# sekelle/SPH-EXA

Measured on AMD Instinct MI355X. Metric: particle-updates/sec (whole node), Sedov -n 400 and Evrard+gravity -n 200, higher is better.
Workload: dtype fp64 coordinates + fp32 hydro (reference precision mix); 1 GPU; model=sedov -n 400 --prop ve (64000000 particles), global_batch=64000000, seq_len=1, parallelism=sfc-domain-decomposition x1, ranks=1, backend=none, leaf_capacity=512

## Files before the change

### sphexa_amd/csrc/hip/bind_hip.cpp

```cpp
#include <array>
#include <stdexcept>
#include <vector>

#include <pybind11/pybind11.h>
#include <pybind11/stl.h>

#include "hip_api.h"

namespace py = pybind11;
using namespace sphx;
using namespace sphx::hip;

namespace
{
using BoxArr   = std::array<double, 9>;
using ConstArr = std::array<double, 16>;
using Ptr      = uintptr_t;

template<class T>
T* P(Ptr p)
{
    return reinterpret_cast<T*>(p);
}

// ... 322 lines not shown
    m.def("chunk_cap", []() { return kChunkCap; });
    m.def("packed_table_region", [](int64_t groups, unsigned ngmax) { return packedTableRegion(groups, ngmax); });

    m.def("xmass",
          [](int64_t first, int64_t last, const ConstArr& c, const BoxArr& box, Ptr nidx, Ptr nc, Ptr x, Ptr y, Ptr z,
             Ptr h, Ptr mm, Ptr wh, Ptr xm, int64_t ntot, Ptr rec, Ptr s, int inDone, Ptr out)
          {
              auto sc = toConsts(c);
              xmass(nbr(first, last, nidx, nc, sc), sc, toBox(box), ntot, P<double>(x), P<double>(y), P<double>(z),
                    P<float>(h), P<float>(mm), P<float>(wh), P<void>(rec), P<float>(xm), St(s), inDone, P<void>(out));
          },
          py::arg("first"), py::arg("last"), py::arg("c"), py::arg("box"), py::arg("nidx"), py::arg("nc"),
          py::arg("x"), py::arg("y"), py::arg("z"), py::arg("h"), py::arg("mm"), py::arg("wh"), py::arg("xm"),
          py::arg("ntot"), py::arg("rec"), py::arg("s"), py::arg("inDone") = 0, py::arg("out") = 0);
    m.def("ve_def_gradh",
          [](int64_t first, int64_t last, const ConstArr& c, const BoxArr& box, Ptr nidx, Ptr nc, Ptr x, Ptr y, Ptr z,
             Ptr h, Ptr mm, Ptr wh, Ptr whd, Ptr xm, Ptr kx, Ptr gradh, int64_t ntot, Ptr rec, Ptr s, double mUniform,
             int inDone, Ptr out, Ptr vx, Ptr vy, Ptr vz, Ptr eosTemp, Ptr eosPrho, Ptr eosC, Ptr eosRho, Ptr eosP)
          {
              auto sc = toConsts(c);
              veDefGradh(nbr(first, last, nidx, nc, sc), sc, toBox(box), ntot, P<double>(x), P<double>(y),
                         P<double>(z), P<float>(h), P<float>(mm), P<float>(wh), P<float>(whd), P<float>(xm),
                         P<void>(rec), P<float>(kx), P<float>(gradh), float(mUniform), St(s), inDone, P<void>(out),
                         P<float>(vx), P<float>(vy), P<float>(vz), P<double>(eosTemp), P<float>(eosPrho),
                         P<float>(eosC), P<float>(eosRho), P<float>(eosP));
          },
          py::arg("first"), py::arg("last"), py::arg("c"), py::arg("box"), py::arg("nidx"), py::arg("nc"),
          py::arg("x"), py::arg("y"), py::arg("z"), py::arg("h"), py::arg("mm"), py::arg("wh"), py::arg("whd"),
          py::arg("xm"), py::arg("kx"), py::arg("gradh"), py::arg("ntot"), py::arg("rec"), py::arg("s"),
          py::arg("mUniform"), py::arg("inDone") = 0, py::arg("out") = 0, py::arg("vx") = 0, py::arg("vy") = 0,
          py::arg("vz") = 0, py::arg("eosTemp") = 0, py::arg("eosPrho") = 0, py::arg("eosC") = 0,
          py::arg("eosRho") = 0, py::arg("eosP") = 0);
    m.def("set_staged", [](unsigned mask) { setStaged(mask); },
          "pair loops that run LDS-staged: bit 0 XMass, 1 Gradh, 2 IAD, 3 AV, 4 momentum (hydro.hip, staged.h)");
    m.def("staged_mask", []() { return stagedMask(); });
    m.def("set_list_masks", [](bool on) { setListMasks(on); },
          "store the per-slot staged-source masks in the list tables even without a staged loop (tests)");
    m.def("set_pair_paths", [](bool kernelFixed, bool momBuf) { setPairPaths(kernelFixed, momBuf); },
          "pair-loop instances: the compile-time sinc^6 kernel function and the momentum loop's 32-bit buffer gathers "
          "(defaults on; tests compare them with the generic instances)", py::arg("kernel_fixed"), py::arg("mom_buf"));
    m.def("set_pair_block", [](int block) { setPairBlock(block); },
          "threads per block of the fixed-point pair loops: 512 (8 target groups sharing a CU's L1) or 256");
    m.def("eos_ve", [](int64_t first, int64_t last, const ConstArr& c, Ptr temp, Ptr mm, Ptr kx, Ptr xm, Ptr gradh,
                       Ptr prho, Ptr cc, Ptr rho, Ptr p, Ptr s)
          {
              eosVe(first, last, toConsts(c), P<double>(temp), P<float>(mm), P<float>(kx), P<float>(xm),
                    P<float>(gradh), P<float>(prho), P<float>(cc), P<float>(rho), P<float>(p), St(s));
          });
    m.def("eos_polytropic", [](int64_t first, int64_t last, Ptr kx, Ptr xm, Ptr mm, Ptr p, Ptr c, Ptr s)
          { eosPolytropic(first, last, P<float>(kx), P<float>(xm), P<float>(mm), P<float>(p), P<float>(c), St(s)); });
    m.def("eos_std", [](int64_t first, int64_t last, const ConstArr& c, Ptr temp, Ptr mm, Ptr rho, Ptr p, Ptr cc,
                        Ptr s)
          {
              eosStd(first, last, toConsts(c), P<double>(temp), P<float>(mm), P<float>(rho), P<float>(p),
                     P<float>(cc), St(s));
          });
    m.def("iad", [](int64_t first, int64_t last, const ConstArr& c, const BoxArr& box, Ptr nidx, Ptr nc, Ptr x, Ptr y,
                    Ptr z, Ptr h, Ptr wh, Ptr numer, Ptr denom, const std::array<Ptr, 6>& cij, int64_t ntot, Ptr rec,
                    Ptr s)
          {
              auto sc = toConsts(c);
              auto cp = six(cij);
              iad(nbr(first, last, nidx, nc, sc), sc, toBox(box), ntot, P<double>(x), P<double>(y), P<double>(z),
                  P<float>(h), P<float>(wh), P<float>(numer), P<float>(denom), P<void>(rec), cp.data(), St(s));
          });
    m.def("iad_divv_curlv",
          [](int64_t first, int64_t last, const ConstArr& c, const BoxArr& box, Ptr nidx, Ptr nc, Ptr x, Ptr y, Ptr z,
             Ptr vx, Ptr vy, Ptr vz, Ptr h, const std::array<Ptr, 6>& cij, Ptr wh, Ptr kx, Ptr xm, Ptr divv,
             Ptr curlv, const std::array<Ptr, 6>& dV, int64_t ntot, Ptr rec, Ptr s, Ptr avS, int inDone, Ptr avOut,
             Ptr momOut, Ptr cs, Ptr mm, Ptr prho, int momSplit)
// ... 270 lines not shown
```

### sphexa_amd/csrc/hip/hip_api.h

```cpp
#pragma once

#include <cstdint>
#include <vector>

#include <hip/hip_runtime.h>

#include "sphx/box.hpp"
#include "sphx/cooling.hpp"
#include "sphx/sph_math.hpp"

namespace sphx::hip
{

struct NsTree
{
    const int32_t* child;
    const int32_t* n2l;
    const int32_t* ns;
    const int32_t* ne;
    const double* center;
    const double* half;
};

struct NbrArgs
// ... 107 lines not shown
void leafBoxesFused(const int32_t* n2l, int64_t N, const int32_t* ns, const int32_t* ne, const double* x,
                    const double* y, const double* z, const int32_t* child, const int32_t* parents, double* center,
                    double* half, unsigned* cnt, hipStream_t s);
void leafBoxes(const int32_t* n2l, int64_t N, const int32_t* ns, const int32_t* ne, const double* x,
               const double* y, const double* z, const float* h, double factor, double* center, double* half,
               hipStream_t s);
void upsweepBoxes(int64_t a, int64_t b, const int32_t* n2l, const int32_t* child, double* center, double* half,
                  hipStream_t s);
void markInBoxes(int64_t nb, const double* bc, const double* bh, const int32_t* child, const int32_t* n2l,
                 const int32_t* ns, const int32_t* ne, const double* center, const double* half, const double* x,
                 const double* y, const double* z, const Box& box, uint8_t* flags, hipStream_t s);

size_t neighborScratchBytes(int64_t n, unsigned ngmax);
struct SplitPredict
{
    const uint64_t* keys = nullptr;
    const unsigned long long* predIn = nullptr;
    unsigned long long* predOut = nullptr;
    int32_t* flags = nullptr;
    int stamp = 0;
    int cap = 0;
    unsigned long long* listCount = nullptr;
    int32_t* list = nullptr;
    int mark = 1;
};
void findNeighbors(int64_t first, int64_t last, const double* x, const double* y, const double* z, float* h,
                   const NsTree& t, const Box& box, unsigned ng0, unsigned ngmax, int32_t* nidx, int home,
                   int ovStride, int32_t* nc, int iterateH, unsigned long long* stats, void* scratch,
                   int testFrontCap, const float* m, int64_t ntot, void* rec, hipStream_t s, const SplitPredict& sp = SplitPredict{});
void setPairBlock(int block);
void setPairPaths(bool kernelFixed, bool momBuf);
void setStaged(unsigned mask);
unsigned stagedMask();
void setListMasks(bool on);
bool listMasksForced();
void packPosQ(int64_t n, const double* x, const double* y, const double* z, const float* m, const QFrame& q,
              SrcPosQ* out, hipStream_t s);
int neighborRowStripes();
void rowPlan(int64_t groups, unsigned ngmax, const int32_t* tab, int home, unsigned long long* over, hipStream_t s);

struct MomFields
{
    const double *x, *y, *z;
    const float *vx, *vy, *vz, *h, *m, *prho, *c;
    const float* cij[6];
    const float *kx, *xm, *alpha;
    const float* dV[6];
};

struct StdFields
{
    const double *x, *y, *z;
    const float *vx, *vy, *vz, *h, *m, *rho, *p, *c;
    const float* cij[6];
};

void xmass(const NbrArgs& a, const SphConsts& sc, const Box& box, int64_t ntot, const double* x, const double* y,
           const double* z, const float* h, const float* m, const float* wh, void* rec, float* xm, hipStream_t s,
           int inDone = 0, void* xmOut = nullptr);
void veDefGradh(const NbrArgs& a, const SphConsts& sc, const Box& box, int64_t ntot, const double* x,
                const double* y, const double* z, const float* h, const float* m, const float* wh, const float* whd,
                const float* xm, void* rec, float* kx, float* gradh, float mUniform, hipStream_t s, int inDone = 0,
                void* iadOut = nullptr, const float* vx = nullptr, const float* vy = nullptr,
                const float* vz = nullptr, const double* eosTemp = nullptr, float* eosPrho = nullptr,
                float* eosC = nullptr, float* eosRho = nullptr, float* eosP = nullptr);
void eosPolytropic(int64_t first, int64_t last, const float* kx, const float* xm, const float* m, float* p, float* c,
                   hipStream_t s);
// ... 106 lines not shown
```

### sphexa_amd/csrc/hip/hydro.hip

```cpp
#include <cfloat>
#include <cstdlib>
#include <type_traits>

#include "common.h"
#include "hip_api.h"
#include "sphx/sph_math.hpp"
#include "staged.h"

namespace sphx::hip
{

#ifndef SPHX_PAIR_BLOCK
#define SPHX_PAIR_BLOCK 256
#endif
constexpr int kBlock = SPHX_PAIR_BLOCK;

template<int B = kBlock>
__device__ __forceinline__ bool targetOf(const NbrArgs& a, int64_t& i, PackedLane& pl, unsigned& n)
{
    __shared__ uint32_t ctabAll[B / 64][kChunkCap];
    unsigned lb     = xcdRemap(blockIdx.x, gridDim.x);
    int64_t t       = int64_t(lb) * B + threadIdx.x;
    i               = a.first + t;
    const int64_t g = t >> 6;
// ... 78 lines not shown
{
    return CoopLoader<R>{rec, waveTile<R>(blockTile), unsigned(self)};
}

inline NbrArgs withTot(NbrArgs a, int64_t ntot)
{
    a.ntot = unsigned(ntot);
    return a;
}

inline unsigned gridT(const NbrArgs& a, int block = kBlock) { return gridFor(a.last - a.first, block); }

static int g_pairBlock = kBlock;
#ifndef SPHX_AV_BLOCK
#define SPHX_AV_BLOCK 640
#endif
#ifndef SPHX_GRADH_BLOCK
#define SPHX_GRADH_BLOCK 1024
#endif
#ifndef SPHX_XMASS_BLOCK
#define SPHX_XMASS_BLOCK 1024
#endif
static const unsigned kPairMask = []
{
    const char* e = std::getenv("SPHX_PAIR_MASK");
    return e ? unsigned(std::strtoul(e, nullptr, 0)) : 31u;
}();

void setPairBlock(int block) { g_pairBlock = block == 512 ? 512 : kBlock; }

static unsigned g_staged = []
{
    const char* e = std::getenv("SPHX_STAGED");
    return e ? unsigned(std::strtoul(e, nullptr, 0)) : 0u;
}();

void setStaged(unsigned mask) { g_staged = mask; }
unsigned stagedMask() { return g_staged; }

static bool g_listMasks = false;
void setListMasks(bool on) { g_listMasks = on; }
bool listMasksForced() { return g_listMasks; }

inline unsigned gridStaged(const NbrArgs& a) { return unsigned((a.last - a.first + 63) / 64); }

template<class F>
inline void withPairBlock(F&& f, int loop = 0)
{
    if (g_pairBlock == 512 && ((kPairMask >> loop) & 1u)) f(std::integral_constant<int, 512>{});
    else f(std::integral_constant<int, kBlock>{});
}

template<int L, class F>
inline void withPairBlockL(F&& f, int loop)
{
    if (g_pairBlock == 512 && ((kPairMask >> loop) & 1u)) f(std::integral_constant<int, L>{});
    else f(std::integral_constant<int, kBlock>{});
}


__global__ void packPosKernel(int64_t n, const double* __restrict__ x, const double* __restrict__ y,
                              const double* __restrict__ z, const float* __restrict__ m,
                              const float* __restrict__ xm, SrcPos* __restrict__ out)
{
    int64_t i = int64_t(blockIdx.x) * blockDim.x + threadIdx.x;
    if (i >= n) return;
    SrcPos r;
    r.x    = x[i];
    r.y    = y[i];
    r.z    = z[i];
    r.m    = m[i];
    r.xm   = xm ? xm[i] : 0.f;
    out[i] = r;
}

// ... 425 lines not shown
{
    int64_t i = first + int64_t(blockIdx.x) * blockDim.x + threadIdx.x;
    if (i >= last) return;
    double rhoi = double(m[i]) / rho[i];
    double pi, ci;
    idealGasEOS(temp[i], rhoi, sc.muiConst, sc.gamma, pi, ci);
    rho[i] = float(rhoi);
    p[i]   = float(pi);
    c[i]   = float(ci);
}

struct Six
{
    float* p[6];
};

__global__ __launch_bounds__(kBlock) void iadKernel(NbrArgs a, SphConsts sc, Box box, const float* __restrict__ h,
                                                    const SrcIad* __restrict__ rec, const float* __restrict__ wh,
                                                    Six cij)
{
    __shared__ float4 tile[kBlock / 64 * 64 * CoopLoader<SrcIad>::S];
    int64_t i;
    PackedLane pl;
    unsigned n;
    const bool valid = targetOf(a, i, pl, n);
    float c[6];
    iadJLoop(unsigned(i), sc.K, box, &pl, 0, n, h[i], coopOf(rec, tile, i, a),
             KernelFn{wh, nullptr, sc.sincIndex, sc.kernelChoice}, c);
    if (!valid) return;
    for (int k = 0; k < 6; ++k)
        cij.p[k][i] = c[k];
}

template<bool kAvS, class R, class G, int B = kBlock, int kKf = 0>
__global__ __launch_bounds__(B) void iadDivvCurlvKernel(NbrArgs a, SphConsts sc, G box,
                                                             const float* __restrict__ h,
                                                             const float* __restrict__ kx,
                                                             const R* __restrict__ rec,
                                                             const float* __restrict__ wh, Six cij,
                                                             float* __restrict__ divv, float* __restrict__ curlv,
                                                             Six dV, int doGrad, float4* __restrict__ avS,
                                                             SrcAvV* __restrict__ avOut, SrcMomQ* __restrict__ momOut,
                                                             const float* __restrict__ cs, const float* __restrict__ mm,
                                                             const float* __restrict__ prho,
                                                             SrcMomSide* __restrict__ momSide = nullptr)
{
    __shared__ float4 tile[B / 64 * 64 * CoopLoader<R>::S];
    int64_t i;
    PackedLane pl;
    unsigned n;
    const bool valid = targetOf<B>(a, i, pl, n);
    float c[6], g[6], dvi, cvi, S[3];
    withKernelFn<kKf>(sc, wh, nullptr, [&](const auto& kf) {
        iadDivvCurlvJLoop<kAvS>(unsigned(i), sc.K, box, &pl, 0, n, h[i], kx[i], coopOf(rec, tile, i, a), kf, c, dvi,
                                cvi, g, S);
    });
    if (valid)
    {
        for (int k = 0; k < 6; ++k)
            cij.p[k][i] = c[k];
        divv[i]  = dvi;
        curlv[i] = cvi;
        if constexpr (kAvS) avS[i - a.first] = make_float4(S[0], S[1], S[2], 0.f);
        if (doGrad)
            for (int k = 0; k < 6; ++k)
                dV.p[k][i] = g[k];
    }
    if constexpr (std::is_same_v<R, SrcIadQ>)
    {
        if ((avOut || momOut) && ballot(valid))
        {
            __shared__ float4 stage[B / 64][64 * 5];
            float4* w       = stage[threadIdx.x >> 6];
            const int lane  = threadIdx.x & 63;
            const int64_t i0 = int64_t(__builtin_amdgcn_readfirstlane(int(i - a.first))) + a.first;
            const int nv     = int(min(int64_t(64), int64_t(a.last) - i0));
            const SrcIadQ pi = rec[i];
            const float ci   = cs[i];
            auto flush = [&](float4* dst, int chunks)
            {
                __builtin_amdgcn_fence(__ATOMIC_RELEASE, "wavefront");
                __builtin_amdgcn_wave_barrier();
                __builtin_amdgcn_fence(__ATOMIC_ACQUIRE, "wavefront");
                for (int q = 0; q < chunks; ++q)
                {
                    const int cidx = q * 64 + lane;
                    if (cidx < nv * chunks) dst[cidx] = w[cidx];
                }
                __builtin_amdgcn_fence(__ATOMIC_RELEASE, "wavefront");
                __builtin_amdgcn_wave_barrier();
                __builtin_amdgcn_fence(__ATOMIC_ACQUIRE, "wavefront");
            };
            if (momOut && momSide)
            {
                SrcMomQ64 r;
                r.x    = pi.x;
                r.y    = pi.y;
                r.z    = pi.z;
                r.vx   = pi.vx;
                r.vy   = pi.vy;
                r.vz   = pi.vz;
                r.ih   = 1.0f / h[i];
                r.c11  = c[0];
                r.c12  = c[1];
                r.c13  = c[2];
                r.c22  = c[3];
// ... 20 lines not shown
                r.vz    = pi.vz;
                r.ih    = 1.0f / h[i];
                r.c11   = c[0];
                r.c12   = c[1];
                r.c13   = c[2];
                r.c22   = c[3];
                r.c23   = c[4];
                r.c33   = c[5];
                r.m     = mm[i];
                r.c     = ci;
                r.xm    = pi.xm;
                r.rho   = kx[i] * r.m / pi.xm;
                r.prho  = prho[i];
                r.alpha = 0.f;
                r.mrho  = r.m / r.rho;
                const float4* rp = reinterpret_cast<const float4*>(&r);
#pragma unroll
                for (int k = 0; k < 5; ++k)
                    w[lane * 5 + k] = rp[k];
                flush(reinterpret_cast<float4*>(momOut + i0), 5);
            }
            if (avOut)
            {
                const SrcAvV r{pi.x, pi.y, pi.z, pi.vol * dvi, pi.vx, pi.vy, pi.vz, ci};
                const float4* rp = reinterpret_cast<const float4*>(&r);
                w[lane * 2]      = rp[0];
                w[lane * 2 + 1]  = rp[1];
                flush(reinterpret_cast<float4*>(avOut + i0), 2);
            }
        }
    }
}

__global__ __launch_bounds__(kBlock) void avSwitchesKernel(NbrArgs a, SphConsts sc, Box box,
                                                           const float* __restrict__ h, Six cij,
                                                           const SrcIad* __restrict__ rec,
                                                           const float* __restrict__ wh, double dt,
                                                           const float* __restrict__ alpha,
                                                           float* __restrict__ alphaOut, const double* dtDev)
{
    __shared__ float4 tile[kBlock / 64 * 64 * CoopLoader<SrcIad>::S];
    int64_t i;
    PackedLane pl;
    unsigned n;
    const bool valid = targetOf(a, i, pl, n);
    if (dtDev) dt = *dtDev;
    float ci[6] = {cij.p[0][i], cij.p[1][i], cij.p[2][i], cij.p[3][i], cij.p[4][i], cij.p[5][i]};
    float al    = avSwitchesJLoop(unsigned(i), sc.K, box, &pl, 0, n, h[i], ci, coopOf(rec, tile, i, a),
                                  KernelFn{wh, nullptr, sc.sincIndex, sc.kernelChoice}, dt, sc.alphamin, sc.alphamax,
                                  sc.decayConstant, alpha[i]);
    if (valid) alphaOut[i] = al;
}

__global__ __launch_bounds__(kBlock) void avSwitchesQKernel(NbrArgs a, SphConsts sc, QFrame q,
                                                            const float* __restrict__ h, Six cij,
                                                            const SrcAvQ* __restrict__ rec,
                                                            const float* __restrict__ divv,
                                                            const float* __restrict__ wh, double dt,
                                                            const float* __restrict__ alpha,
                                                            float* __restrict__ alphaOut, const double* dtDev)
{
    int64_t i;
    PackedLane pl;
    unsigned n;
    const bool valid = targetOf(a, i, pl, n);
    if (dtDev) dt = *dtDev;
    float ci[6] = {cij.p[0][i], cij.p[1][i], cij.p[2][i], cij.p[3][i], cij.p[4][i], cij.p[5][i]};
    float al    = avSwitchesJLoop(unsigned(i), sc.K, q, &pl, 0, n, h[i], ci, AvQLoader{rec, divv},
                                  KernelFn{wh, nullptr, sc.sincIndex, sc.kernelChoice}, dt, sc.alphamin, sc.alphamax,
                                  sc.decayConstant, alpha[i]);
    if (valid) alphaOut[i] = al;
}

template<int B = kBlock, int kKf = 0>
__global__ __launch_bounds__(B) void avSwitchesVKernel(NbrArgs a, SphConsts sc, QFrame q,
                                                            const float* __restrict__ h, Six cij,
                                                            const SrcAvV* __restrict__ rec,
                                                            const float* __restrict__ divv,
                                                            const float4* __restrict__ avS,
                                                            const float* __restrict__ wh, double dt,
                                                            const float* __restrict__ alpha,
                                                            float* __restrict__ alphaOut, const double* dtDev,
                                                            SrcMomQ* __restrict__ momOut,
                                                            SrcMomSide* __restrict__ momSide = nullptr)
{
    __shared__ float4 tile[B / 64 * 64 * CoopLoader<SrcAvV>::S];
    int64_t i;
    PackedLane pl;
    unsigned n;
    const bool valid = targetOf<B>(a, i, pl, n);
    if (dtDev) dt = *dtDev;
    float ci[6]    = {cij.p[0][i], cij.p[1][i], cij.p[2][i], cij.p[3][i], cij.p[4][i], cij.p[5][i]};
    const float4 s = avS[i - a.first];
    const float S[3] = {s.x, s.y, s.z};
    float al;
    withKernelFn<kKf>(sc, wh, nullptr, [&](const auto& kf) {
        al = avSwitchesVJLoop(unsigned(i), sc.K, q, &pl, 0, n, h[i], ci, divv[i], S, coopOf(rec, tile, i, a), kf, dt,
                              sc.alphamin, sc.alphamax, sc.decayConstant, alpha[i]);
    });
    if (!valid) return;
    alphaOut[i] = al;
    if (momSide) momSide[i].alpha = al;
    else if (momOut) momOut[i].alpha = al;
}

template<int B = kBlock>
__device__ inline void reduceMinDt(float dti, float* minDt)
{
    __shared__ float red[B / 64];
    float v = waveMin(dti);
    int w   = threadIdx.x >> 6;
    if ((threadIdx.x & 63) == 0) red[w] = v;
    __syncthreads();
    if (threadIdx.x == 0)
    {
        float r = red[0];
        for (int k = 1; k < B / 64; ++k)
            r = fminf(r, red[k]);
        atomicMinPosFloat(minDt, r);
    }
}

struct GradVLoader
{
    const SrcGradV* r;
    __device__ SrcGradV operator()(unsigned j) const
    {
        if (r) return r[j];
        SrcGradV g{};
        return g;
// ... 450 lines not shown
    return reinterpret_cast<SrcMomSide*>(static_cast<char*>(momOut) + momSideOffset(ntot));
}

void iadDivvCurlv(const NbrArgs& a, const SphConsts& sc, const Box& box, int64_t ntot, const double* x,
                  const double* y, const double* z, const float* vx, const float* vy, const float* vz, const float* h,
                  const float* wh, const float* kx, const float* xm, void* rec, float* const cij[6], float* divv,
                  float* curlv, float* const dV[6], void* avS, hipStream_t s, int inDone, void* avOut, void* momOut,
                  const float* cs, const float* m, const float* prho, int momSplit)
{
    if (a.last <= a.first) return;
    SrcMomSide* momSide = momSideOf(momOut, ntot, momSplit);
    Six c, g;
    for (int k = 0; k < 6; ++k)
    {
        c.p[k] = cij[k];
        g.p[k] = dV[k];
    }
    if (!sc.fixedPoint)
    {
        packIadKernel<<<gridFor(ntot, 256), 256, 0, s>>>(ntot, x, y, z, xm, kx, vx, vy, vz, xm, nullptr, nullptr,
                                                         (SrcIad*)rec);
        iadDivvCurlvKernel<false><<<gridT(a), kBlock, 0, s>>>(withTot(a, ntot), sc, box, h, kx, (const SrcIad*)rec, wh,
                                                              c, divv, curlv, g, dV[0] != nullptr, nullptr, nullptr,
                                                              nullptr, nullptr, nullptr, nullptr);
    }
    else
    {
        const QFrame q = qframeOf(box, sc.fixedPoint);
        packRanges(inDone, a, ntot, [&](int64_t lo, int64_t hi)
                   {
                       packIadQKernel<<<gridFor(hi - lo, 256), 256, 0, s>>>(lo, hi, x, y, z, kx, vx, vy, vz, xm, q,
                                                                            (SrcIadQ*)rec);
                   });
        withPairBlock([&](auto bc)
                      {
                          constexpr int B = decltype(bc)::value;
                          withKf(sc, [&](auto kk)
                          {
                              constexpr int KK = decltype(kk)::value;
                              if (avS)
                                  iadDivvCurlvKernel<true, SrcIadQ, QFrame, B, KK><<<gridT(a, B), B, 0, s>>>(
                                      withTot(a, ntot), sc, q, h, kx, (const SrcIadQ*)rec, wh, c, divv, curlv, g,
                                      dV[0] != nullptr, (float4*)avS, (SrcAvV*)avOut, (SrcMomQ*)momOut, cs, m, prho,
                                      momSide);
                              else
                                  iadDivvCurlvKernel<false, SrcIadQ, QFrame, B, KK><<<gridT(a, B), B, 0, s>>>(
                                      withTot(a, ntot), sc, q, h, kx, (const SrcIadQ*)rec, wh, c, divv, curlv, g,
                                      dV[0] != nullptr, nullptr, nullptr, (SrcMomQ*)momOut, cs, m, prho, momSide);
                          });
                      }, 2);
    }
    SPHX_LAUNCH_CHECK();
}

void avSwitches(const NbrArgs& a, const SphConsts& sc, const Box& box, int64_t ntot, const double* x,
                const double* y, const double* z, const float* vx, const float* vy, const float* vz, const float* h,
                const float* c, float* const cij[6], const float* wh, const float* kx, const float* xm,
                const float* divv, double dt, void* rec, const void* avS, float* alpha, hipStream_t s, int inDone,
                void* momOut, float* alphaOut, const double* dtDev, int momSplit)
{
    if (!alphaOut) alphaOut = alpha;
    if (a.last <= a.first) return;
    Six cc;
    for (int k = 0; k < 6; ++k)
        cc.p[k] = cij[k];
    if (!sc.fixedPoint)
    {
        packIadKernel<<<gridFor(ntot, 256), 256, 0, s>>>(ntot, x, y, z, xm, kx, vx, vy, vz, xm, c, divv, (SrcIad*)rec);
        avSwitchesKernel<<<gridT(a), kBlock, 0, s>>>(withTot(a, ntot), sc, box, h, cc, (const SrcIad*)rec, wh, dt, alpha,
                                                      alphaOut, dtDev);
    }
    else if (avS)
    {
        const QFrame q = qframeOf(box, sc.fixedPoint);
        packRanges(inDone, a, ntot, [&](int64_t lo, int64_t hi)
                   {
                       packAvVKernel<<<gridFor(hi - lo, 256), 256, 0, s>>>(lo, hi, x, y, z, kx, vx, vy, vz, xm, c, divv,
                                                                           q, (SrcAvV*)rec);
                   });
        withPairBlockL<SPHX_AV_BLOCK>([&](auto bc)
                      {
                          constexpr int B = decltype(bc)::value;
                          withKf(sc, [&](auto kk)
                                 {
                                     avSwitchesVKernel<B, decltype(kk)::value><<<gridT(a, B), B, 0, s>>>(
                                         withTot(a, ntot), sc, q, h, cc, (const SrcAvV*)rec, divv, (const float4*)avS,
                                         wh, dt, alpha, alphaOut, dtDev, (SrcMomQ*)momOut,
                                         momSideOf(momOut, ntot, momSplit));
                                 });
                      }, 3);
    }
    else
    {
        const QFrame q = qframeOf(box, sc.fixedPoint);
        packAvQKernel<<<gridFor(ntot, 256), 256, 0, s>>>(ntot, x, y, z, kx, vx, vy, vz, xm, c, q, (SrcAvQ*)rec);
        avSwitchesQKernel<<<gridT(a), kBlock, 0, s>>>(withTot(a, ntot), sc, q, h, cc, (const SrcAvQ*)rec, divv, wh, dt,
                                                      alpha, alphaOut, dtDev);
    }
    SPHX_LAUNCH_CHECK();
}

void momentumEnergyVe(const NbrArgs& a, const SphConsts& sc, const Box& box, int64_t ntot, const MomFields& f,
                      bool avClean, const float* wh, void* rec, void* recGradV, float* ax, float* ay, float* az,
                      double* du, float* minDt, hipStream_t s, int inDone, float mUniform)
{
    if (a.last <= a.first) return;
    if (sc.fixedPoint && mUniform > 0.f && !avClean)
    {
        if (reinterpret_cast<uintptr_t>(rec) & 63) throw std::invalid_argument("momentum records: 64-B alignment");
        const QFrame q  = qframeOf(box, sc.fixedPoint);
        auto* main      = static_cast<SrcMomQ64*>(rec);
        auto* side      = reinterpret_cast<SrcMomSide*>(static_cast<char*>(rec) + momSideOffset(ntot));
// ... 108 lines not shown
```

### sphexa_amd/csrc/hip/neighbors.hip

```cpp
#include <type_traits>

#include "common.h"
#include "hip_api.h"
#include "sphx/box.hpp"
#include "sphx/packed_list.hpp"
#include "sphx/sph_math.hpp"

namespace sphx::hip
{

#ifndef SPHX_NS_WPB
#define SPHX_NS_WPB 1
#endif
constexpr int kWavesPerBlock = SPHX_NS_WPB;
constexpr int kFrontCap      = 512;
#ifndef SPHX_NS_LEAFCAP
#define SPHX_NS_LEAFCAP 256
#endif
#ifndef SPHX_NS_ROUNDED
#define SPHX_NS_ROUNDED 1
#endif
#ifndef SPHX_NS_DOT
#define SPHX_NS_DOT 1
#endif
// ... 998 lines not shown
    SideStream& st = side[dev & 63];
    if (!st.s)
    {
        int lo = 0, hi = 0;
        SPHX_CHECK(hipDeviceGetStreamPriorityRange(&lo, &hi));
        SPHX_CHECK(hipStreamCreateWithPriority(&st.s, hipStreamNonBlocking, hi));
        SPHX_CHECK(hipEventCreateWithFlags(&st.fork, hipEventDisableTiming));
        SPHX_CHECK(hipEventCreateWithFlags(&st.join, hipEventDisableTiming));
    }
    return st;
}
}

void findNeighbors(int64_t first, int64_t last, const double* x, const double* y, const double* z, float* h,
                   const NsTree& t, const Box& box, unsigned ng0, unsigned ngmax, int32_t* nidx, int home,
                   int ovStride, int32_t* nc, int iterateH, unsigned long long* stats, void* scratch,
                   int testFrontCap, const float* m, int64_t ntot, void* rec, hipStream_t s, const SplitPredict& sp)
{
    int64_t n = last - first;
    if (n <= 0) return;
    int64_t groups = (n + 63) / 64;
    if (packedTableInts(ngmax) > 64 || home < 0 || ovStride < 1)
        throw std::invalid_argument("findNeighbors: ngmax too large for packed lists or bad row pool");
    const unsigned long long ovBase = (unsigned long long)groups * home;
    const PackedOut po{nidx,
                       reinterpret_cast<int4*>(nidx + packedTableRegion(groups, ngmax)),
                       packedRowsMax(ngmax),
                       packedTableInts(ngmax),
                       unsigned(home),
                       unsigned(ovStride),
                       ovBase,
                       ovBase + (unsigned long long)kRowStripes * ovStride,
                       stats + 8,
                       stagedMask() != 0u || listMasksForced() ? 1 : 0};
    int64_t spillMemOff, total;
    scratchLayout(n, spillMemOff, total);
    int32_t* splitList = static_cast<int32_t*>(scratch);
    int32_t* spillList = splitList + spillMemOff / 2;
    int32_t* spillMem  = splitList + spillMemOff;
    const int fc       = testFrontCap > 0 ? min(testFrontCap, kFrontCap) : kFrontCap;
    const unsigned grid = unsigned((groups + kWavesPerBlock - 1) / kWavesPerBlock);
    const QFrame qf     = qframeOf(box);
    SrcPosQ* xq         = static_cast<SrcPosQ*>(rec);
    packPosQ(ntot, x, y, z, m, qf, xq, s);
    const bool record  = sp.keys && sp.predIn && sp.predOut && sp.flags && sp.list && sp.cap > 0;
    const bool predict = record && sp.mark;
    const PredOut pout{sp.keys, record ? sp.predOut : nullptr, sp.cap, fc};
    SideStream* side = predict ? &sideStream() : nullptr;
    auto launch = [&](auto capped)
    {
        constexpr bool kC = decltype(capped)::value;
        const int fcs = testFrontCap > 0 ? min(testFrontCap, kSplitFront) : kSplitFront;
        if (record) SPHX_CHECK(hipMemsetAsync(sp.predOut, 0, sizeof(unsigned long long), s));
        if (predict)
        {
            SPHX_CHECK(hipMemsetAsync(sp.listCount, 0, sizeof(unsigned long long), s));
            predMarkKernel<<<1, 256, 0, s>>>(sp.keys, first, last, sp.predIn, sp.cap, sp.flags, sp.stamp,
                                             sp.listCount, sp.list, stats);
            SPHX_LAUNCH_CHECK();
            SPHX_CHECK(hipEventRecord(side->fork, s));
            SPHX_CHECK(hipStreamWaitEvent(side->s, side->fork, 0));
            findNeighborsSplitKernel<kC><<<kSplitWaves, 64, 0, side->s>>>(first, last, x, y, z, xq, qf, uint32_t(ntot), h,
                                                                           t, box, ng0, ngmax, po, nc, iterateH, stats,
                                                                           sp.list, sp.listCount, spillList, fcs,
                                                                           pout);
            SPHX_LAUNCH_CHECK();
            SPHX_CHECK(hipEventRecord(side->join, side->s));
// ... 21 lines not shown
```

### sphexa_amd/csrc/hip/staged.h

```cpp
#pragma once

#include "common.h"
#include "sphx/packed_list.hpp"
#include "sphx/sph_math.hpp"

namespace sphx::hip
{

constexpr int kStRows = 64;

template<int UCAP, int RC, bool kSide>
struct StagedShared
{
    float4 rec[UCAP * RC];
    float2 side[kSide ? UCAP : 1];
    uint32_t jl[UCAP];
    uint16_t pos[kStRows * 64];
    uint32_t c0[kStRows];
    uint32_t base[kStRows];
    uint32_t mlo[kStRows], mhi[kStRows];
    int win[2];
};

struct StagedLane
// ... 275 lines not shown
            float t = s[(k * W) * 64 + lane];
#pragma unroll
            for (int ww = 1; ww < W; ++ww)
                t += s[(k * W + ww) * 64 + lane];
            v[k] = t;
        }
    }
}

template<class R, int W, int UCAP, bool kSide, class... T>
__device__ void reduceAcrossMax(const StagedLoader<R, W, UCAP, kSide>& ld, T&... v)
{
    if constexpr (W > 1)
    {
        float* s            = reinterpret_cast<float*>(ld.sh->rec);
        const unsigned lane = threadIdx.x & 63, w = threadIdx.x >> 6;
        __syncthreads();
        int k = 0;
        ((s[(k++ * W + w) * 64 + lane] = float(v)), ...);
        __syncthreads();
        k          = 0;
        auto total = [&](int kk)
        {
            float t = s[(kk * W) * 64 + lane];
#pragma unroll
            for (int ww = 1; ww < W; ++ww)
                t = fmaxf(t, s[(kk * W + ww) * 64 + lane]);
            return t;
        };
        ((v = total(k++)), ...);
    }
}

}
```

### sphexa_amd/ops/neighbors.py

```python

from __future__ import annotations

import os
from dataclasses import dataclass

import numpy as np
import torch

from . import _lib
from .reduce import zero_
from .sfc import gather
from .octree import Octree
from ..utils.box import Box

GROUP = 64


def _stream():
    return _lib.stream()


@dataclass
class NeighborList:
    nidx: torch.Tensor
# ... 127 lines not shown
class NeighborSearchError(RuntimeError):
    pass


_SCRATCH: dict = {}
TEST_FRONT_CAP = 0
TEST_FORCE_SPLIT = False
COLLECT_STATS = os.environ.get("SPHX_SEARCH_STATS") == "1"
SPLIT_LEN = {"64": 0, "32": 8, "16": 16}[os.environ.get("SPHX_SPLIT_LEN", "64")]
ALLOW_NC_FAIL = os.environ.get("SPHX_ALLOW_NC_FAIL") == "1"


def _check_convergence(d, fails: int):
    d._h_min = None
    d._h_min_global = None
    d._h_max_global = None
    d.nc_fail = int(fails)
    if fails > 0 and not ALLOW_NC_FAIL:
        raise NeighborSearchError(f"coupled nc/h iteration failed to converge ({fails} particles on the CPU path, target groups on the GPU) "
                                  f"(ng0={d.ng0}, ngmax={d.ngmax}); set SPHX_ALLOW_NC_FAIL=1 to continue anyway")


def _scratch(nbytes: int, device, key: str = "") -> torch.Tensor:
    t = _SCRATCH.get((device, key))
    if t is None or t.numel() < nbytes:
        t = torch.empty(nbytes, dtype=torch.uint8, device=device)
        _SCRATCH[(device, key)] = t
    return t


def _pool_plan(prev: NeighborList | None, groups: int, ng0: int, stripes: int):
    if prev is not None and prev.grouped and prev.plan is not None and prev.plan[0] == groups:
        return prev.plan[1], prev.plan[2]
    masks = 1 if _lib.hip().staged_mask() else 0
    return max(1, round(ng0 / 8) + 1 + masks), max(8, -(-int(0.35 * ng0 / 8 * groups + 0.5) // stripes))


_STATS_IDX: dict = {}


def _stats_index(K: int, device) -> torch.Tensor:
    key = (K, device)
    t = _STATS_IDX.get(key)
    if t is None:
        t = _STATS_IDX[key] = torch.tensor(list(range(8)) + [8 + 32 * k for k in range(K)], dtype=torch.int32,
                                           device=device)
    return t


SPLIT_PREDICT = os.environ.get("SPHX_SPLIT_PREDICT", "1") == "1"
PRED_CAP = 1024


class _PredState:

    def __init__(self, device):
        self.rec = [zero_(torch.empty(1 + 2 * PRED_CAP, dtype=torch.int64, device=device)) for _ in range(2)]
        self.plist = torch.empty(1 + (3 * PRED_CAP + 1) // 2, dtype=torch.int64, device=device)
        self.flags = None
        self.stamp = 0
        self.cur = 0
        self.active = True

    def args(self, groups: int, device) -> dict:
        if self.flags is None or self.flags.numel() < groups:
            self.flags = zero_(torch.empty(max(groups, 1024) * 5 // 4, dtype=torch.int32, device=device))
        self.stamp = self.stamp % (2**31 - 2) + 1
# ... 169 lines not shown
```

Measured before the change: 579.7 million particle-updates/s.

## Stage block-wide neighbor-record unions in LDS for IAD and AV loops

Adds block-union kernels for the IAD/divv-curlv and AV-switch pair loops. Each block hashes the source chunks of its target groups into LDS, deduplicates them, and copies the union of needed records into shared memory once. The neighbor loop then reads records from LDS instead of making per-wave global gathers. It falls back to the gathered loop when the union overflows capacity or the slot masks are missing. The default staged mask changes to enable IAD and AV, which forces the neighbor search to store slot masks, and the IAD epilogue reuses the record LDS for its row staging.

```diff
diff --git a/sphexa_amd/csrc/hip/bind_hip.cpp b/sphexa_amd/csrc/hip/bind_hip.cpp
--- a/sphexa_amd/csrc/hip/bind_hip.cpp
+++ b/sphexa_amd/csrc/hip/bind_hip.cpp
@@ -378,10 +378,16 @@
           py::arg("vz") = 0, py::arg("eosTemp") = 0, py::arg("eosPrho") = 0, py::arg("eosC") = 0,
           py::arg("eosRho") = 0, py::arg("eosP") = 0);
     m.def("set_staged", [](unsigned mask) { setStaged(mask); },
-          "pair loops that run LDS-staged: bit 0 XMass, 1 Gradh, 2 IAD, 3 AV, 4 momentum (hydro.hip, staged.h)");
+          "pair loops that run LDS-staged: bit 0 XMass, 1 Gradh, 2 IAD, 3 AV, 4 momentum, 5 IAD and AV also on 256-thread "
+          "blocks (hydro.hip, staged.h)");
     m.def("staged_mask", []() { return stagedMask(); });
+    m.def("set_staged_counters", [](Ptr counters) { setStagedCounters(P<unsigned>(counters)); },
+          "two uint32 device counters of the block-union loops (blocks staged, blocks fallen back to the gathered "
+          "loop); 0: not counted (production)");
     m.def("set_list_masks", [](bool on) { setListMasks(on); },
           "store the per-slot staged-source masks in the list tables even without a staged loop (tests)");
+    m.def("list_masks_wanted", []() { return listMasksWanted(); },
+          "whether the search stores the slot masks: forced, or read by a staged loop of this run");
     m.def("set_pair_paths", [](bool kernelFixed, bool momBuf) { setPairPaths(kernelFixed, momBuf); },
           "pair-loop instances: the compile-time sinc^6 kernel function and the momentum loop's 32-bit buffer gathers "
           "(defaults on; tests compare them with the generic instances)", py::arg("kernel_fixed"), py::arg("mom_buf"));
diff --git a/sphexa_amd/csrc/hip/hip_api.h b/sphexa_amd/csrc/hip/hip_api.h
--- a/sphexa_amd/csrc/hip/hip_api.h
+++ b/sphexa_amd/csrc/hip/hip_api.h
@@ -163,7 +163,9 @@
 void setPairPaths(bool kernelFixed, bool momBuf);
 void setStaged(unsigned mask);
 unsigned stagedMask();
+void setStagedCounters(unsigned* counters);
 void setListMasks(bool on);
+bool listMasksWanted();
 bool listMasksForced();
 void packPosQ(int64_t n, const double* x, const double* y, const double* z, const float* m, const QFrame& q,
               SrcPosQ* out, hipStream_t s);
diff --git a/sphexa_amd/csrc/hip/hydro.hip b/sphexa_amd/csrc/hip/hydro.hip
--- a/sphexa_amd/csrc/hip/hydro.hip
+++ b/sphexa_amd/csrc/hip/hydro.hip
@@ -134,15 +134,37 @@
 static unsigned g_staged = []
 {
     const char* e = std::getenv("SPHX_STAGED");
-    return e ? unsigned(std::strtoul(e, nullptr, 0)) : 0u;
+    return e ? unsigned(std::strtoul(e, nullptr, 0)) : 12u;
 }();
 
 void setStaged(unsigned mask) { g_staged = mask; }
 unsigned stagedMask() { return g_staged; }
+
+static bool unionLoopOn(int loop)
+{
+    const bool big = g_pairBlock == 512 && ((kPairMask >> loop) & 1u);
+    return ((g_staged >> loop) & 1u) && (big || (g_staged & 32u));
+}
+
+static unsigned* g_stagedCounters = nullptr;
+void setStagedCounters(unsigned* counters) { g_stagedCounters = counters; }
+
+#ifndef SPHX_STB_U512
+#define SPHX_STB_U512 2264
+#endif
+#ifndef SPHX_STB_U256
+#define SPHX_STB_U256 1128
+#endif
+template<int B>
+constexpr int kUnionCap = B == 512 ? SPHX_STB_U512 : SPHX_STB_U256;
+static_assert(sizeof(BlockUnionShared<8, kUnionCap<512>, 2>) * 2 <= 160 * 1024 &&
+                  sizeof(BlockUnionShared<4, kUnionCap<256>, 2>) * 4 <= 160 * 1024,
+              "16 waves per CU with the unions in LDS");
 
 static bool g_listMasks = false;
 void setListMasks(bool on) { g_listMasks = on; }
 bool listMasksForced() { return g_listMasks; }
+bool listMasksWanted() { return g_listMasks || (g_staged & 1u) || unionLoopOn(2) || unionLoopOn(3); }
 
 inline unsigned gridStaged(const NbrArgs& a) { return unsigned((a.last - a.first + 63) / 64); }
 
@@ -634,29 +656,16 @@
         cij.p[k][i] = c[k];
 }
 
-template<bool kAvS, class R, class G, int B = kBlock, int kKf = 0>
-__global__ __launch_bounds__(B) void iadDivvCurlvKernel(NbrArgs a, SphConsts sc, G box,
-                                                             const float* __restrict__ h,
-                                                             const float* __restrict__ kx,
-                                                             const R* __restrict__ rec,
-                                                             const float* __restrict__ wh, Six cij,
-                                                             float* __restrict__ divv, float* __restrict__ curlv,
-                                                             Six dV, int doGrad, float4* __restrict__ avS,
-                                                             SrcAvV* __restrict__ avOut, SrcMomQ* __restrict__ momOut,
-                                                             const float* __restrict__ cs, const float* __restrict__ mm,
-                                                             const float* __restrict__ prho,
-                                                             SrcMomSide* __restrict__ momSide = nullptr)
-{
-    __shared__ float4 tile[B / 64 * 64 * CoopLoader<R>::S];
-    int64_t i;
-    PackedLane pl;
-    unsigned n;
-    const bool valid = targetOf<B>(a, i, pl, n);
-    float c[6], g[6], dvi, cvi, S[3];
-    withKernelFn<kKf>(sc, wh, nullptr, [&](const auto& kf) {
-        iadDivvCurlvJLoop<kAvS>(unsigned(i), sc.K, box, &pl, 0, n, h[i], kx[i], coopOf(rec, tile, i, a), kf, c, dvi,
-                                cvi, g, S);
-    });
+template<bool kAvS, class R>
+__device__ __forceinline__ void iadEpilogue(const NbrArgs& a, bool valid, int64_t i, const float* __restrict__ h,
+                                            const float* __restrict__ kx, const R* __restrict__ rec, Six cij,
+                                            float* __restrict__ divv, float* __restrict__ curlv, Six dV, int doGrad,
+                                            float4* __restrict__ avS, SrcAvV* __restrict__ avOut,
+                                            SrcMomQ* __restrict__ momOut, const float* __restrict__ cs,
+                                            const float* __restrict__ mm, const float* __restrict__ prho,
+                                            SrcMomSide* __restrict__ momSide, const float (&c)[6], const float (&g)[6],
+                                            float dvi, float cvi, const float (&S)[3], float4* w)
+{
     if (valid)
     {
         for (int k = 0; k < 6; ++k)
@@ -672,8 +681,6 @@
     {
         if ((avOut || momOut) && ballot(valid))
         {
-            __shared__ float4 stage[B / 64][64 * 5];
-            float4* w       = stage[threadIdx.x >> 6];
             const int lane  = threadIdx.x & 63;
             const int64_t i0 = int64_t(__builtin_amdgcn_readfirstlane(int(i - a.first))) + a.first;
             const int nv     = int(min(int64_t(64), int64_t(a.last) - i0));
@@ -760,6 +767,73 @@
     }
 }
 
+template<bool kAvS, class R, class G, int B = kBlock, int kKf = 0>
+__global__ __launch_bounds__(B) void iadDivvCurlvKernel(NbrArgs a, SphConsts sc, G box,
+                                                             const float* __restrict__ h,
+                                                             const float* __restrict__ kx,
+                                                             const R* __restrict__ rec,
+                                                             const float* __restrict__ wh, Six cij,
+                                                             float* __restrict__ divv, float* __restrict__ curlv,
+                                                             Six dV, int doGrad, float4* __restrict__ avS,
+                                                             SrcAvV* __restrict__ avOut, SrcMomQ* __restrict__ momOut,
+                                                             const float* __restrict__ cs, const float* __restrict__ mm,
+                                                             const float* __restrict__ prho,
+                                                             SrcMomSide* __restrict__ momSide = nullptr)
+{
+    __shared__ float4 tile[B / 64 * 64 * CoopLoader<R>::S];
+    int64_t i;
+    PackedLane pl;
+    unsigned n;
+    const bool valid = targetOf<B>(a, i, pl, n);
+    float c[6], g[6], dvi, cvi, S[3];
+    withKernelFn<kKf>(sc, wh, nullptr, [&](const auto& kf) {
+        iadDivvCurlvJLoop<kAvS>(unsigned(i), sc.K, box, &pl, 0, n, h[i], kx[i], coopOf(rec, tile, i, a), kf, c, dvi,
+                                cvi, g, S);
+    });
+    float4* w = nullptr;
+    if constexpr (std::is_same_v<R, SrcIadQ>)
+    {
+        __shared__ float4 stage[B / 64][64 * 5];
+        w = stage[threadIdx.x >> 6];
+    }
+    iadEpilogue<kAvS>(a, valid, i, h, kx, rec, cij, divv, curlv, dV, doGrad, avS, avOut, momOut, cs, mm, prho, momSide,
+                      c, g, dvi, cvi, S, w);
+}
+
+template<bool kAvS, int B, int kKf, int UCAP>
+__global__ __launch_bounds__(B) void iadDivvCurlvUnionKernel(NbrArgs a, SphConsts sc, QFrame box,
+                                                             const float* __restrict__ h,
+                                                             const float* __restrict__ kx,
+                                                             const SrcIadQ* __restrict__ rec,
+                                                             const float* __restrict__ wh, Six cij,
+                                                             float* __restrict__ divv, float* __restrict__ curlv,
+                                                             Six dV, int doGrad, float4* __restrict__ avS,
+                                                             SrcAvV* __restrict__ avOut, SrcMomQ* __restrict__ momOut,
+                                                             const float* __restrict__ cs, const float* __restrict__ mm,
+                                                             const float* __restrict__ prho,
+                                                             SrcMomSide* __restrict__ momSide, unsigned* counters)
+{
+    using Ld = BlockUnionLoader<SrcIadQ, B / 64, UCAP>;
+    __shared__ typename Ld::Shared sh;
+    static_assert(sizeof(sh.rec) >= sizeof(float4) * (B / 64) * 64 * 5, "the epilogue's rows fit the records' LDS");
+    int64_t i;
+    PackedLane pl;
+    BlockLane bl;
+    unsigned n;
+    const bool valid  = blockTargetOf<B>(a, i, pl, n, bl);
+    const bool staged = stageBlockUnion<SrcIadQ, B / 64, UCAP>(bl, rec, a.ntot, sh, counters);
+    if (!staged) loadChunkTable(bl, pl, sh);
+    float c[6], g[6], dvi, cvi, S[3];
+    withKernelFn<kKf>(sc, wh, nullptr, [&](const auto& kf) {
+        iadDivvCurlvJLoop<kAvS>(unsigned(i), sc.K, box, &pl, 0, n, h[i], kx[i], Ld{rec, &sh, &bl, staged}, kf, c, dvi,
+                                cvi, g, S);
+    });
+    __syncthreads();
+    float4* w = reinterpret_cast<float4*>(sh.rec) + (threadIdx.x >> 6) * 64 * 5;
+    iadEpilogue<kAvS>(a, valid, i, h, kx, rec, cij, divv, curlv, dV, doGrad, avS, avOut, momOut, cs, mm, prho, momSide,
+                      c, g, dvi, cvi, S, w);
+}
+
 __global__ __launch_bounds__(kBlock) void avSwitchesKernel(NbrArgs a, SphConsts sc, Box box,
                                                            const float* __restrict__ h, Six cij,
                                                            const SrcIad* __restrict__ rec,
@@ -824,6 +898,42 @@
     float al;
     withKernelFn<kKf>(sc, wh, nullptr, [&](const auto& kf) {
         al = avSwitchesVJLoop(unsigned(i), sc.K, q, &pl, 0, n, h[i], ci, divv[i], S, coopOf(rec, tile, i, a), kf, dt,
+                              sc.alphamin, sc.alphamax, sc.decayConstant, alpha[i]);
+    });
+    if (!valid) return;
+    alphaOut[i] = al;
+    if (momSide) momSide[i].alpha = al;
+    else if (momOut) momOut[i].alpha = al;
+}
+
+template<int B, int kKf, int UCAP>
+__global__ __launch_bounds__(B) void avSwitchesVUnionKernel(NbrArgs a, SphConsts sc, QFrame q,
+                                                            const float* __restrict__ h, Six cij,
+                                                            const SrcAvV* __restrict__ rec,
+                                                            const float* __restrict__ divv,
+                                                            const float4* __restrict__ avS,
+                                                            const float* __restrict__ wh, double dt,
+                                                            const float* __restrict__ alpha,
+                                                            float* __restrict__ alphaOut, const double* dtDev,
+                                                            SrcMomQ* __restrict__ momOut,
+                                                            SrcMomSide* __restrict__ momSide, unsigned* counters)
+{
+    using Ld = BlockUnionLoader<SrcAvV, B / 64, UCAP>;
+    __shared__ typename Ld::Shared sh;
+    int64_t i;
+    PackedLane pl;
+    BlockLane bl;
+    unsigned n;
+    const bool valid  = blockTargetOf<B>(a, i, pl, n, bl);
+    const bool staged = stageBlockUnion<SrcAvV, B / 64, UCAP>(bl, rec, a.ntot, sh, counters);
+    if (!staged) loadChunkTable(bl, pl, sh);
+    if (dtDev) dt = *dtDev;
+    float ci[6]    = {cij.p[0][i], cij.p[1][i], cij.p[2][i], cij.p[3][i], cij.p[4][i], cij.p[5][i]};
+    const float4 s = avS[i - a.first];
+    const float S[3] = {s.x, s.y, s.z};
+    float al;
+    withKernelFn<kKf>(sc, wh, nullptr, [&](const auto& kf) {
+        al = avSwitchesVJLoop(unsigned(i), sc.K, q, &pl, 0, n, h[i], ci, divv[i], S, Ld{rec, &sh, &bl, staged}, kf, dt,
                               sc.alphamin, sc.alphamax, sc.decayConstant, alpha[i]);
     });
     if (!valid) return;
@@ -1340,6 +1450,29 @@
                        packIadQKernel<<<gridFor(hi - lo, 256), 256, 0, s>>>(lo, hi, x, y, z, kx, vx, vy, vz, xm, q,
                                                                             (SrcIadQ*)rec);
                    });
+        if (unionLoopOn(2))
+        {
+            withPairBlock([&](auto bc)
+                          {
+                              constexpr int B = decltype(bc)::value;
+                              withKf(sc, [&](auto kk)
+                              {
+                                  constexpr int KK = decltype(kk)::value;
+                                  if (avS)
+                                      iadDivvCurlvUnionKernel<true, B, KK, kUnionCap<B>><<<gridT(a, B), B, 0, s>>>(
+                                          withTot(a, ntot), sc, q, h, kx, (const SrcIadQ*)rec, wh, c, divv, curlv, g,
+                                          dV[0] != nullptr, (float4*)avS, (SrcAvV*)avOut, (SrcMomQ*)momOut, cs, m, prho,
+                                          momSide, g_stagedCounters);
+                                  else
+                                      iadDivvCurlvUnionKernel<false, B, KK, kUnionCap<B>><<<gridT(a, B), B, 0, s>>>(
+                                          withTot(a, ntot), sc, q, h, kx, (const SrcIadQ*)rec, wh, c, divv, curlv, g,
+                                          dV[0] != nullptr, nullptr, nullptr, (SrcMomQ*)momOut, cs, m, prho, momSide,
+                                          g_stagedCounters);
+                              });
+                          }, 2);
+            SPHX_LAUNCH_CHECK();
+            return;
+        }
         withPairBlock([&](auto bc)
                       {
                           constexpr int B = decltype(bc)::value;
@@ -1386,6 +1519,23 @@
                        packAvVKernel<<<gridFor(hi - lo, 256), 256, 0, s>>>(lo, hi, x, y, z, kx, vx, vy, vz, xm, c, divv,
                                                                            q, (SrcAvV*)rec);
                    });
+        if (unionLoopOn(3))
+        {
+            withPairBlock([&](auto bc)
+                          {
+                              constexpr int B = decltype(bc)::value;
+                              withKf(sc, [&](auto kk)
+                                     {
+                                         avSwitchesVUnionKernel<B, decltype(kk)::value, kUnionCap<B>>
+                                             <<<gridT(a, B), B, 0, s>>>(
+                                                 withTot(a, ntot), sc, q, h, cc, (const SrcAvV*)rec, divv,
+                                                 (const float4*)avS, wh, dt, alpha, alphaOut, dtDev, (SrcMomQ*)momOut,
+                                                 momSideOf(momOut, ntot, momSplit), g_stagedCounters);
+                                     });
+                          }, 3);
+            SPHX_LAUNCH_CHECK();
+            return;
+        }
         withPairBlockL<SPHX_AV_BLOCK>([&](auto bc)
                       {
                           constexpr int B = decltype(bc)::value;
diff --git a/sphexa_amd/csrc/hip/neighbors.hip b/sphexa_amd/csrc/hip/neighbors.hip
--- a/sphexa_amd/csrc/hip/neighbors.hip
+++ b/sphexa_amd/csrc/hip/neighbors.hip
@@ -1054,7 +1054,7 @@
                        ovBase,
                        ovBase + (unsigned long long)kRowStripes * ovStride,
                        stats + 8,
-                       stagedMask() != 0u || listMasksForced() ? 1 : 0};
+                       listMasksWanted() ? 1 : 0};
     int64_t spillMemOff, total;
     scratchLayout(n, spillMemOff, total);
     int32_t* splitList = static_cast<int32_t*>(scratch);
diff --git a/sphexa_amd/csrc/hip/staged.h b/sphexa_amd/csrc/hip/staged.h
--- a/sphexa_amd/csrc/hip/staged.h
+++ b/sphexa_amd/csrc/hip/staged.h
@@ -331,4 +331,277 @@
     }
 }
 
-}
+
+constexpr unsigned kBuSlots = 64;
+constexpr uint32_t kBuEmpty = 0xFFFFFFFFu;
+
+struct BlockLane
+{
+    const int32_t* tab;
+    const int32_t* rowsInt;
+    unsigned nch, Tc, T;
+    unsigned gfirst;
+
+    __device__ __forceinline__ int32_t rowOf(unsigned o) const
+    {
+        return *(const __attribute__((address_space(4))) int32_t*)(tab + 2 + o);
+    }
+};
+
+template<int NG, int UCAP, int RC>
+struct BlockUnionShared
+{
+    static constexpr int HS = 64 * NG;
+    union
+    {
+        uint4 rec[(UCAP + 1) * RC];
+        uint32_t ctab[NG][kChunkCap];
+    };
+    uint4 tab[HS];
+    uint16_t dense[HS];
+    unsigned wsum[NG];
+    unsigned fail;
+};
+
+template<int B>
+__device__ __forceinline__ bool blockTargetOf(const NbrArgs& a, int64_t& i, PackedLane& pl, unsigned& n, BlockLane& bl)
+{
+    const unsigned lb   = xcdRemap(blockIdx.x, gridDim.x);
+    const int64_t t     = int64_t(lb) * B + threadIdx.x;
+    i                   = a.first + t;
+    const int64_t g     = t >> 6;
+    const int64_t G     = (a.last - a.first + 63) / 64;
+    const unsigned lane = threadIdx.x & 63;
+    bl.tab              = a.nidx + g * int64_t(packedTableInts(a.ngmax));
+    bl.rowsInt          = a.nidx + packedTableRegion(G, a.ngmax);
+    bl.nch = bl.Tc = bl.T = 0;
+    bl.gfirst             = unsigned(a.first + g * 64);
+    pl.nblk               = 0;
+    if (g < G)
+    {
+        pl.nblk          = unsigned(*(const __attribute__((address_space(4))) int32_t*)(bl.tab));
+        const unsigned w = unsigned(*(const __attribute__((address_space(4))) int32_t*)(bl.tab + 1));
+        bl.nch           = min(tableWordNch(w), kChunkCap);
+        bl.Tc            = tableWordTc(w);
+        bl.T             = tableWordT(w);
+    }
+    pl.tab  = bl.tab + 2 + bl.T;
+    pl.rows = reinterpret_cast<const int4*>(bl.rowsInt) + lane;
+    pl.ctab = nullptr;
+#ifdef SPHX_DEVICE_CHECKS
+    pl.ntot = a.ntot;
+    SPHX_DCHECK(pl.nblk <= listBlocksMax(a.ngmax), 1);
+    pl.nblk = min(pl.nblk, listBlocksMax(a.ngmax));
+#endif
+    if (i >= a.last)
+    {
+        i       = a.last - 1;
+        pl.self = unsigned(i);
+        n       = 0;
+        return false;
+    }
+    pl.self = unsigned(i);
+    const int cnt = a.nc[i] - 1;
+    n             = unsigned(cnt < 0 ? 0 : (unsigned(cnt) < a.ngmax ? cnt : a.ngmax));
+    return true;
+}
+
+template<int NG, int UCAP, int RC>
+__device__ __forceinline__ void loadChunkTable(const BlockLane& bl, PackedLane& pl, BlockUnionShared<NG, UCAP, RC>& sh)
+{
+    const unsigned lane = threadIdx.x & 63;
+    uint32_t* ctab      = sh.ctab[threadIdx.x >> 6];
+    for (unsigned e = lane; e < bl.nch; e += 64)
+        ctab[e] = uint32_t(bl.rowsInt[size_t(bl.rowOf(e >> 8)) * 256 + (e & 255)]);
+    asm volatile("s_waitcnt vmcnt(0) lgkmcnt(0)" ::: "memory");
+    pl.ctab = ctab;
+}
+
+template<class R, int NG, int UCAP>
+__device__ bool stageBlockUnion(const BlockLane& bl, const R* __restrict__ rec, unsigned ntot,
+                                BlockUnionShared<NG, UCAP, int(sizeof(R) / 16)>& sh, unsigned* counters)
+{
+    constexpr int RC = int(sizeof(R) / 16);
+    constexpr int HS = 64 * NG;
+    static_assert((HS & (HS - 1)) == 0, "hash size is a power of two");
+    static_assert(UCAP + 64 < 65536 && NG * (kBuSlots - 1) * 64 < 65536, "the scan packs two 16-bit counts");
+    const unsigned t = threadIdx.x, lane = t & 63, wave = t >> 6;
+    sh.tab[t] = make_uint4(kBuEmpty, 0u, 0u, 0u);
+    if (t == 0) sh.fail = 0u;
+    __syncthreads();
+    const bool masks  = bl.T >= bl.Tc + maskTabRows(bl.nch) && bl.T > bl.Tc;
+    const bool waveOk = bl.nch <= kBuSlots && (bl.nch <= 1u || masks);
+    const bool mine   = waveOk && lane >= 1u && lane < bl.nch;
+    bool bad          = !waveOk;
+    unsigned e        = 0;
+    if (mine)
+    {
+        const uint32_t cb = uint32_t(bl.rowsInt[size_t(bl.rowOf(0)) * 256 + lane]);
+        const int32_t* mr = bl.rowsInt + size_t(bl.rowOf(bl.Tc)) * 256 + 2 * lane;
+        uint32_t lo = uint32_t(mr[0]), hi = uint32_t(mr[1]);
+        if (cb >= ntot) bad = true;
+        else
+        {
+            const unsigned avail = min(ntot - cb, 64u);
+            const uint64_t keep  = avail >= 64u ? ~0ull : ((1ull << avail) - 1ull);
+            lo &= uint32_t(keep);
+            hi &= uint32_t(keep >> 32);
+            unsigned hsh = (cb * 2654435761u) >> (32 - __builtin_ctz(unsigned(HS)));
+            bool done    = false;
+            for (int tries = 0; tries < HS && !done; ++tries)
+            {
+                const uint32_t old = atomicCAS(&sh.tab[hsh].x, kBuEmpty, cb);
+                if (old == kBuEmpty || old == cb)
+                {
+                    if (lo) atomicOr(&sh.tab[hsh].z, lo);
+                    if (hi) atomicOr(&sh.tab[hsh].w, hi);
+                    e    = hsh;
+                    done = true;
+                }
+                else hsh = (hsh + 1u) & unsigned(HS - 1);
+            }
+            if (!done) bad = true;
+        }
+    }
+    if (bad) sh.fail = 1u;
+    __syncthreads();
+    uint4 ent          = sh.tab[t];
+    const bool used    = ent.x != kBuEmpty;
+    const unsigned cnt = used ? unsigned(__popc(ent.z) + __popc(ent.w)) : 0u;
+    const unsigned pk  = cnt | (used ? 1u << 16 : 0u);
+    unsigned incl      = pk;
+#pragma unroll
+    for (int o = 1; o < 64; o <<= 1)
+    {
+        const unsigned up = unsigned(__shfl_up(int(incl), o));
+        if (int(lane) >= o) incl += up;
+    }
+    if (lane == 63) sh.wsum[wave] = incl;
+    __syncthreads();
+    unsigned before = 0, total = 0;
+#pragma unroll
+    for (int w = 0; w < NG; ++w)
+    {
+        const unsigned s = sh.wsum[w];
+        before += unsigned(w) < wave ? s : 0u;
+        total += s;
+    }
+    const unsigned excl = before + incl - pk;
+    const unsigned nrec = total & 0xFFFFu, nent = total >> 16;
+    const bool staged   = sh.fail == 0u && nrec <= unsigned(UCAP);
+    if (counters && t == 0) atomicAdd(&counters[staged ? 0 : 1], 1u);
+    if (!staged)
+    {
+        __syncthreads();
+        return false;
+    }
+    if (used)
+    {
+        sh.tab[t].y               = excl & 0xFFFFu;
+        sh.dense[excl >> 16]      = uint16_t(t);
+    }
+    __syncthreads();
+    uint4 slotEnt = make_uint4(bl.gfirst, 0u, 0u, 0u);
+    if (mine) slotEnt = sh.tab[e];
+    for (unsigned k = wave; k < nent; k += NG)
+    {
+        const uint4 en   = sh.tab[sh.dense[k]];
+        const uint64_t m = uint64_t(en.w) << 32 | en.z;
+        if ((m >> lane) & 1)
+        {
+            const unsigned p = en.y + unsigned(__popcll(m & lanemaskLt()));
+            const uint4* src = reinterpret_cast<const uint4*>(rec) + size_t(en.x + lane) * RC;
+#pragma unroll
+            for (int c = 0; c < RC; ++c)
+                sh.rec[p * RC + c] = src[c];
+        }
+    }
+    __syncthreads();
+    sh.tab[t] = slotEnt;
+    __syncthreads();
+    return true;
+}
+
+template<class R, int NG, int UCAP, class F>
+__device__ void forEachNeighborUnion(const PackedLane& pl, const BlockLane& bl,
+                                     const BlockUnionShared<NG, UCAP, int(sizeof(R) / 16)>& sh, F&& f)
+{
+    constexpr int RC    = int(sizeof(R) / 16);
+    const unsigned nblk = pl.nblk;
+    if (nblk == 0) return;
+    const uint4* wtab = sh.tab + (threadIdx.x >> 6) * 64;
+    int4 w            = pl.block(0);
+    auto batch = [&](int w0, int w1)
+    {
+        const uint32_t ws[2] = {uint32_t(w0), uint32_t(w1)};
+        unsigned j[4];
+        R rr[4];
+#pragma unroll
+        for (int u = 0; u < 4; ++u)
+        {
+            const uint32_t code = (ws[u >> 1] >> ((u & 1) * 16)) & 0xFFFFu;
+            const unsigned slot = code & (kBuSlots - 1u), off = code >> kChunkSlotBits;
+            const uint4 en      = wtab[slot];
+            const uint32_t below = (1u << (off & 31u)) - 1u;
+            const bool upper     = off >= 32u;
+            const uint32_t lo = upper ? en.z : en.z & below, hi = upper ? en.w & below : 0u;
+            unsigned p        = en.y + unsigned(__popc(lo)) + unsigned(__popc(hi));
+            j[u]              = en.x + off;
+#ifdef SPHX_DEVICE_CHECKS
+            const bool ok = (code & kChunkSlotMask) < max(bl.nch, 1u) && p < unsigned(UCAP) &&
+                            ((code & kChunkSlotMask) != 0u || j[u] == pl.self);
+            SPHX_DCHECK(ok, 0);
+            if (!ok)
+            {
+                p    = 0u;
+                j[u] = pl.self;
+            }
+#endif
+            uint4 o4[RC];
+#pragma unroll
+            for (int c = 0; c < RC; ++c)
+                o4[c] = sh.rec[p * RC + c];
+            float4 o[RC];
+#pragma unroll
+            for (int c = 0; c < RC; ++c)
+                o[c] = make_float4(__uint_as_float(o4[c].x), __uint_as_float(o4[c].y), __uint_as_float(o4[c].z),
+                                   __uint_as_float(o4[c].w));
+            rr[u] = stagedUnpack<R>(o);
+        }
+#pragma unroll
+        for (int u = 0; u < 4; ++u)
+        {
+            pinRegs(rr[u]);
+            if (j[u] != pl.self) f(j[u], rr[u]);
+        }
+    };
+    for (unsigned b = 0; b < nblk; ++b)
+    {
+        const int4 wn = pl.block(b + 1);
+        batch(w.x, w.y);
+        batch(w.z, w.w);
+        w = wn;
+    }
+    (void)bl;
+}
+
+template<class R, int NG, int UCAP>
+struct BlockUnionLoader
+{
+    using Shared = BlockUnionShared<NG, UCAP, int(sizeof(R) / 16)>;
+    const R* r;
+    const Shared* sh;
+    const BlockLane* bl;
+    bool staged;
+
+    __device__ R operator()(unsigned j) const { return r[j]; }
+};
+
+template<int B, class R, int NG, int UCAP, class F>
+__device__ void forEachNeighbor(const PackedLane* pl, int, unsigned, const BlockUnionLoader<R, NG, UCAP>& ld, F&& f)
+{
+    if (ld.staged) forEachNeighborUnion<R, NG, UCAP>(*pl, *ld.bl, *ld.sh, f);
+    else forEachNeighborDirect(*pl, ld, f);
+}
+
+}
diff --git a/sphexa_amd/ops/neighbors.py b/sphexa_amd/ops/neighbors.py
--- a/sphexa_amd/ops/neighbors.py
+++ b/sphexa_amd/ops/neighbors.py
@@ -183,7 +183,7 @@
 def _pool_plan(prev: NeighborList | None, groups: int, ng0: int, stripes: int):
     if prev is not None and prev.grouped and prev.plan is not None and prev.plan[0] == groups:
         return prev.plan[1], prev.plan[2]
-    masks = 1 if _lib.hip().staged_mask() else 0
+    masks = 1 if _lib.hip().list_masks_wanted() else 0
     return max(1, round(ng0 / 8) + 1 + masks), max(8, -(-int(0.35 * ng0 / 8 * groups + 0.5) // stripes))
 
 
```

Result: faster. 613.0 million particle-updates/s (median of 6 runs) (+5.7%).
